# nju-ee/MODE-2022

Measured on AMD Instinct MI355X. Metric: ERP stereo pairs/sec (512x1024, 192 disp) fwd+bwd, higher is better.
Workload: dtype fp32 storage/accumulate; products: 2xfp16 split (22-bit, per-tensor 2^k scale, 3 MFMAs) in the stride-1 3x3x3 / spherical / 3x3 layers incl. gradients (DESIGN 3u/3v); 3xbf16 split (24-bit, 6 MFMAs) in the stride-2 / transposed 3x3x3 layers and the polar spherical tiles (3j-3l); fp32 MFMA in the 32->; 1 GPU; ModeDisparity(192,Sphere,1024x512 Cassini) fwd+bwd+Adam step, batch 2/GPU (BASELINE configs[2]); global_batch=2, conv_arith=bf16x6, init=recipe state, seed 1 (tests/golden/recipe.py), parallelism=dp1

## Files before the change

mode-2022_amd/csrc/conv2d_split_wgrad.hip:

```cpp
#include "common.h"

#include "bn_internal.h"
#include "conv3d_internal.h"
#include "split_arith.h"

namespace {

using namespace mode::split;

constexpr int NT = 256;
constexpr int RING = 12;
constexpr int XROWP = 40;
constexpr int XPIECE = RING * XROWP;
constexpr int XCS = 3 * XPIECE + 8;
constexpr int XALL = 32 * XCS;
constexpr int GPIECE = 4 * 32;
constexpr int GCS = 3 * GPIECE + 8;
constexpr int GBUF = 32 * GCS;
constexpr size_t TILE_BYTES = (size_t)(XALL + 2 * GBUF) * 2;
constexpr size_t SUM_BYTES = (size_t)3 * 9 * 1024 * sizeof(float);
constexpr size_t LDS_BYTES = TILE_BYTES > SUM_BYTES ? TILE_BYTES : SUM_BYTES;
constexpr int GIT = 32 * 4 * 16 / NT;

template <int DIL, bool F16>
__global__ __launch_bounds__(NT) void conv2d_bww_split_kernel(const float* __restrict__ gy, const float* __restrict__ x,
                                                              float* __restrict__ part, mode::Wgrad2SplitDims d,
                                                              const float* __restrict__ amax_g, const float* __restrict__ amax_x) {
  constexpr int NPC = Arith<F16>::NP;
  float sg = 1.f, sx = 1.f, unscale = 1.f;
  if (F16) {
    sg = f16_scale_of(mode::absmax_load(amax_g));
    sx = f16_scale_of(mode::absmax_load(amax_x));
    unscale = (1.f / sg) * (1.f / sx);
  }
  constexpr int NP = (32 + 2 * DIL) / 2;
  constexpr int XIT = (32 * 4 * NP + NT - 1) / NT;
  extern __shared__ __attribute__((aligned(16))) uint16_t lds[];
  uint16_t* xl = lds;
  uint16_t* gl = lds + XALL;
  const int s = blockIdx.x, ob = blockIdx.y, cb = blockIdx.z;
  const int tid = threadIdx.x, wave = tid >> 6, lane = tid & 63, half = lane >> 5;
  const int HWi = d.H * d.W;

  f32x16 acc[9];
#pragma unroll
  for (int t = 0; t < 9; ++t) acc[t] = (f32x16){0};

  int x_c[XIT], x_row[XIT], x_wp[XIT], g_o[GIT], g_row[GIT], g_wp[GIT];
#pragma unroll
  for (int k = 0; k < XIT; ++k) {
    const int item = min(tid + k * NT, 32 * 4 * NP - 1);
    x_wp[k] = item % NP;
    x_row[k] = (item / NP) % 4;
    x_c[k] = item / (NP * 4);
  }
#pragma unroll
  for (int k = 0; k < GIT; ++k) {
    const int item = tid + k * NT;
    g_wp[k] = item % 16;
    g_row[k] = (item / 16) % 4;
    g_o[k] = item / 64;
  }
  const float* xb = x;
  const float* gb = gy;
  float xr[XIT][2], gr[GIT][2];
  constexpr unsigned kHalfOOB = 0x40000000u;
  unsigned xo0[XIT], xo1[XIT], go0[GIT], go1[GIT];
  int xdst[XIT], gdst[GIT];
#pragma unroll
  for (int k = 0; k < XIT; ++k) xdst[k] = x_c[k] * XCS + 2 * x_wp[k];
#pragma unroll
  for (int k = 0; k < GIT; ++k) gdst[k] = g_o[k] * GCS + g_row[k] * 32 + 2 * g_wp[k];
  auto unit_begin = [&](int w0) {
#pragma unroll
    for (int k = 0; k < XIT; ++k) {
      const int gw = w0 - DIL + 2 * x_wp[k];
      const unsigned cok = (unsigned)(cb * 32 + x_c[k] < d.Ci);
      const unsigned base = 4u * (unsigned)(x_c[k] * HWi + x_row[k] * d.W + gw);
      xo0[k] = (cok & (unsigned)((unsigned)gw < (unsigned)d.W)) ? base : kHalfOOB;
      xo1[k] = (cok & (unsigned)((unsigned)(gw + 1) < (unsigned)d.W)) ? base + 4u : kHalfOOB;
    }
#pragma unroll
    for (int k = 0; k < GIT; ++k) {
      const int gw = w0 + 2 * g_wp[k];
      const unsigned ook = (unsigned)(ob * 32 + g_o[k] < d.Co);
      const unsigned base = 4u * (unsigned)(g_o[k] * HWi + g_row[k] * d.W + gw);
      go0[k] = (ook & (unsigned)(gw < d.W)) ? base : kHalfOOB;
      go1[k] = (ook & (unsigned)(gw + 1 < d.W)) ? base + 4u : kHalfOOB;
    }
  };
  const unsigned block_bytes = 128u * (unsigned)HWi;
  auto load_x = [&](int k, int r0) {
    const __amdgpu_buffer_rsrc_t rs = buf_rsrc(xb, block_bytes);
    const unsigned ro = (unsigned)(r0 + x_row[k]) < (unsigned)d.H ? (unsigned)(4 * r0 * d.W) : kHalfOOB;
    xr[k][0] = buf_load_f32(rs, xo0[k] + ro, 0);
    xr[k][1] = buf_load_f32(rs, xo1[k] + ro, 0);
  };
  auto commit_x = [&](int k, int r0, int slot0) {
    uint32_t p1, p2, p3;
    const float v0 = xr[k][0], v1 = xr[k][1];
    int sl = slot0 + x_row[k];
    sl = sl >= RING ? sl - RING : sl;
    uint32_t* dst = reinterpret_cast<uint32_t*>(xl + xdst[k] + sl * XROWP);
    if constexpr (F16) {
      split2_f16_pinned(v0 * sx, v1 * sx, p1, p2);
    } else {
      split3_bf16_pinned(v0, v1, p1, p2, p3);
      dst[XPIECE] = p3;
    }
    dst[0] = p1;
    dst[XPIECE / 2] = p2;
  };
  auto load_g = [&](int k, int r0) {
    const __amdgpu_buffer_rsrc_t rs = buf_rsrc(gb, block_bytes);
    const unsigned ro = r0 + g_row[k] < d.H ? (unsigned)(4 * r0 * d.W) : kHalfOOB;
    gr[k][0] = buf_load_f32(rs, go0[k] + ro, 0);
    gr[k][1] = buf_load_f32(rs, go1[k] + ro, 0);
  };
  auto commit_g = [&](int k, int r0, int buf) {
    uint32_t p1, p2, p3;
    const float v0 = gr[k][0], v1 = gr[k][1];
    uint32_t* dst = reinterpret_cast<uint32_t*>(gl + buf * GBUF + gdst[k]);
    if constexpr (F16) {
      split2_f16_pinned(v0 * sg, v1 * sg, p1, p2);
    } else {
      split3_bf16_pinned(v0, v1, p1, p2, p3);
      dst[GPIECE] = p3;
    }
    dst[0] = p1;
    dst[GPIECE / 2] = p2;
  };

  for (int u = xcd_remap(s, d.S); u < d.units; u += d.S) {
    int t = u;
    const int run = t % d.nRun;
    t /= d.nRun;
    const int wt = t % d.nWt;
    const int b = t / d.nWt;
    const int g_lo = run * d.run_groups, g_hi = min(d.nGroups, g_lo + d.run_groups);
    xb = x + ((long long)b * d.Ci + cb * 32) * HWi;
    gb = gy + ((long long)b * d.Co + ob * 32) * HWi;
    unit_begin(wt * 32);

    const int h_first = g_lo * 4;
#pragma unroll 1
    for (int pass = 0; pass < 2; ++pass) {
#pragma unroll
      for (int k = 0; k < XIT; ++k) load_x(k, h_first - DIL + 4 * pass);
#pragma unroll
      for (int k = 0; k < XIT; ++k) commit_x(k, h_first - DIL + 4 * pass, 4 * pass);
    }
#pragma unroll
    for (int k = 0; k < GIT; ++k) load_g(k, h_first);
#pragma unroll
    for (int k = 0; k < GIT; ++k) commit_g(k, h_first, 0);
    lds_barrier();

    int sbase = 0;
#pragma unroll 1
    for (int g = g_lo; g < g_hi; ++g) {
      const int h0 = g * 4, gbuf = (g - g_lo) & 1;
      const int sfront = sbase + 8 >= RING ? sbase + 8 - RING : sbase + 8;
      int xrow[3];
#pragma unroll
      for (int kh = 0; kh < 3; ++kh) {
        int sl = sbase + wave + kh * DIL;
        sl = sl >= RING ? sl - RING : sl;
        xrow[kh] = (lane & 31) * XCS + sl * XROWP + 8 * half;
      }
      const uint16_t* ga = gl + gbuf * GBUF + (lane & 31) * GCS + wave * 32 + 8 * half;
      uint4 ra[2][3], rlo[2][3];
      uint2 rhi[2][3];
      auto read_stage = [&](int i) {
        const int ks = i / 3, kh = i % 3;
#pragma unroll
        for (int p = 0; p < NPC; ++p) {
          if (kh == 0) ra[ks][p] = *reinterpret_cast<const uint4*>(__builtin_assume_aligned(ga + p * GPIECE + 16 * ks, 16));
          const uint32_t* src = reinterpret_cast<const uint32_t*>(__builtin_assume_aligned(xl + xrow[kh] + p * XPIECE + 16 * ks, 16));
          rlo[i & 1][p] = *reinterpret_cast<const uint4*>(src);
          rhi[i & 1][p] = *reinterpret_cast<const uint2*>(src + 4);
        }
      };
      read_stage(0);
#pragma unroll
      for (int i = 0; i < 6; ++i) {
        const int ks = i / 3, kh = i % 3;
        if (i + 1 < 6) read_stage(i + 1);
        if (i < 3) {
#pragma unroll
          for (int k = 3 * i; k < 3 * i + 3; ++k) load_x(k, h0 - DIL + 8);
#pragma unroll
          for (int k = (GIT * i) / 3; k < (GIT * (i + 1)) / 3; ++k) load_g(k, h0 + 4);
          if (!F16) __builtin_amdgcn_sched_barrier(0);
        } else {
#pragma unroll
          for (int k = 3 * (i - 3); k < 3 * (i - 3) + 3; ++k) commit_x(k, h0 - DIL + 8, sfront);
#pragma unroll
          for (int k = (GIT * (i - 3)) / 3; k < (GIT * (i - 2)) / 3; ++k) commit_g(k, h0 + 4, gbuf ^ 1);
        }
        uint4 bq[3][3];
#pragma unroll
        for (int p = 0; p < NPC; ++p) {
          const uint4 lo = rlo[i & 1][p];
          const uint2 hi = rhi[i & 1][p];
          const uint32_t dw[6] = {lo.x, lo.y, lo.z, lo.w, hi.x, hi.y};
          constexpr uint32_t SEL_MID = 0x05040302u, SEL_HI = 0x07060504u;
#pragma unroll
          for (int kw = 0; kw < 3; ++kw) {
            const int sh = kw * DIL;
            if (sh == 0) {
              bq[kw][p] = lo;
            } else {
              const int sd = sh == 4 ? 1 : 0;
              const uint32_t sel = (sh & 1) ? SEL_MID : SEL_HI;
              bq[kw][p] = make_uint4(__builtin_amdgcn_perm(dw[sd + 1], dw[sd], sel), __builtin_amdgcn_perm(dw[sd + 2], dw[sd + 1], sel),
                                     __builtin_amdgcn_perm(dw[sd + 3], dw[sd + 2], sel), __builtin_amdgcn_perm(dw[sd + 4], dw[sd + 3], sel));
            }
          }
        }
        if constexpr (F16) {
#define MODE_SPLIT_TERM(PA, PB) \
  _Pragma("unroll") for (int kw = 0; kw < 3; ++kw) acc[3 * kh + kw] = mfma_f16(ra[ks][PA], bq[kw][PB], acc[3 * kh + kw]);
          MODE_SPLIT_TERM(1, 0)
          MODE_SPLIT_TERM(0, 1)
          MODE_SPLIT_TERM(0, 0)
#undef MODE_SPLIT_TERM
        } else {
#define MODE_SPLIT_TERM(PA, PB) \
  _Pragma("unroll") for (int kw = 0; kw < 3; ++kw) acc[3 * kh + kw] = mfma_bf16(ra[ks][PA], bq[kw][PB], acc[3 * kh + kw]);
          MODE_SPLIT_TERM(2, 0)
          MODE_SPLIT_TERM(0, 2)
          MODE_SPLIT_TERM(1, 1)
          MODE_SPLIT_TERM(1, 0)
          MODE_SPLIT_TERM(0, 1)
          MODE_SPLIT_TERM(0, 0)
#undef MODE_SPLIT_TERM
        }
#pragma unroll
        for (int j = 0; j < (F16 ? 9 : 18); ++j) {
          __builtin_amdgcn_sched_group_barrier(0x008, 1, 0);
          if (F16) {
            __builtin_amdgcn_sched_group_barrier(0x002, 6, 0);
            if (i < 3) {
              __builtin_amdgcn_sched_group_barrier(0x020, 2, 0);
              __builtin_amdgcn_sched_group_barrier(0x080, 1, 0);
            } else {
              __builtin_amdgcn_sched_group_barrier(0x080, 2, 0);
            }
          } else {
            __builtin_amdgcn_sched_group_barrier(0x002, 7, 0);
            __builtin_amdgcn_sched_group_barrier(0x100, 1, 0);
            __builtin_amdgcn_sched_group_barrier(0x200, 2, 0);
          }
        }
        __builtin_amdgcn_sched_barrier(0);
      }
      sbase = sbase + 4 >= RING ? sbase + 4 - RING : sbase + 4;
      lds_barrier();
    }
  }

  float* sums = reinterpret_cast<float*>(lds);
  if (wave > 0) {
#pragma unroll
    for (int tap = 0; tap < 9; ++tap)
#pragma unroll
      for (int q = 0; q < 16; ++q) sums[((wave - 1) * 9 + tap) * 1024 + q * 64 + lane] = acc[tap][q];
  }
  __syncthreads();
  if (wave == 0) {
    float* pb = part + (((long long)s * d.MTo + ob) * d.MTc + cb) * (9 * 1024);
#pragma unroll
    for (int tap = 0; tap < 9; ++tap)
#pragma unroll
      for (int q = 0; q < 16; ++q) {
        const int i = (q & 3) + 8 * (q >> 2) + 4 * half;
        const float v = ((acc[tap][q] + sums[tap * 1024 + q * 64 + lane]) + sums[(9 + tap) * 1024 + q * 64 + lane]) +
                        sums[(18 + tap) * 1024 + q * 64 + lane];
        pb[tap * 1024 + i * 32 + (lane & 31)] = F16 ? v * unscale : v;
      }
  }
}

}

namespace mode {

int conv2d_bww_split_launch(const float* gy, const float* x, float* part, const Wgrad2SplitDims& d, int dilation, hipStream_t st,
                            const char* who, const float* amax_g, const float* amax_x) {
#define MODE_C2W_LAUNCH(DILV, F16V)                                                                                              \
  {                                                                                                                              \
    int rc = allow_lds(conv2d_bww_split_kernel<DILV, F16V>, LDS_BYTES, who);                                                     \
    if (rc != MODE_OK) return rc;                                                                                                \
    hipLaunchKernelGGL((conv2d_bww_split_kernel<DILV, F16V>), dim3(d.S, d.MTo, d.MTc), dim3(NT), LDS_BYTES, st, gy, x, part, d, amax_g, \
                       amax_x);                                                                                                  \
  }
  if (dilation == 1) {
    if (amax_g) MODE_C2W_LAUNCH(1, true) else MODE_C2W_LAUNCH(1, false)
  } else {
    if (amax_g) MODE_C2W_LAUNCH(2, true) else MODE_C2W_LAUNCH(2, false)
  }
#undef MODE_C2W_LAUNCH
  return check_launch(who);
}

}
```

mode-2022_amd/csrc/conv2d_wgrad.hip:

```cpp
#include "common.h"
#include "conv3d_internal.h"

namespace {

typedef float f32x16 __attribute__((ext_vector_type(16)));
constexpr int NT = 256;
constexpr int TH = 4;

__device__ __forceinline__ f32x16 mfma32(float a, float b, f32x16 c) {
  return __builtin_amdgcn_mfma_f32_32x32x2f32(a, b, c, 0, 0, 0);
}

struct W2Dims {
  int B, Ci, Co, H, W;
  int nHt, nWt, T, S, MTo, MTc;
};

template <int DIL>
struct Geo {
  static constexpr int XR = TH + 2 * DIL, XW = 32 + 2 * DIL;
  static constexpr int XPLANE = (XR * XW) | 1;
  static constexpr int GPLANE = TH * 32 + 1;
  static constexpr size_t LDS = (size_t)(32 * XPLANE + 32 * GPLANE) * sizeof(float);
};

template <int DIL>
__global__ __launch_bounds__(NT, 2) void conv2d_bwd_weight_kernel(const float* __restrict__ gy, const float* __restrict__ x,
                                                                  float* __restrict__ part, W2Dims d) {
  using G = Geo<DIL>;
  constexpr int XR = G::XR, XW = G::XW, XPLANE = G::XPLANE, GPLANE = G::GPLANE;
  constexpr int NXM = 4 * XR;
  constexpr int NHALO = 32 * XR * 2 * DIL;
  constexpr int NXH = (NHALO + NT - 1) / NT;
  extern __shared__ __attribute__((aligned(16))) float lds[];
  float* xl = lds;
  float* gl = lds + 32 * XPLANE;
  const int s = blockIdx.x, ob = blockIdx.y, cb = blockIdx.z;
  const int tid = threadIdx.x, wave = tid >> 6, lane = tid & 63;
  const int hwv = tid >> 5, l32 = tid & 31;
  const int HW = d.H * d.W;

  f32x16 acc[9];
#pragma unroll
  for (int t = 0; t < 9; ++t) acc[t] = (f32x16){0};

  float px[NXM], ph[NXH], pg[16];
  unsigned chan_ok = 0, gchan_ok = 0;
#pragma unroll
  for (int q = 0; q < 4; ++q) {
    chan_ok |= (cb * 32 + hwv + 8 * q < d.Ci ? 1u : 0u) << q;
    gchan_ok |= (ob * 32 + hwv + 8 * q < d.Co ? 1u : 0u) << q;
  }

  auto halo_geom = [&](int k, int& c, int& r, int& col) {
    const int e = k * NT + tid;
    const int cr = e / (2 * DIL), j = e - cr * (2 * DIL);
    c = cr / XR;
    r = cr - c * XR;
    col = j < DIL ? j : 32 + j;
    return e < NHALO;
  };

  auto prefetch = [&](int tt, int& h0, int& w0) {
    int t = tt;
    const int wt = t % d.nWt;
    t /= d.nWt;
    const int ht = t % d.nHt;
    const int b = t / d.nHt;
    w0 = wt * 32;
    h0 = ht * TH;
    const float* xb = x + ((long long)b * d.Ci + cb * 32) * (long long)HW;
    const float* gb = gy + ((long long)b * d.Co + ob * 32) * (long long)HW;
    const int gw = w0 + l32;
    const bool wok = gw < d.W;
#pragma unroll
    for (int jj = 0; jj < NXM; ++jj) {
      const int q = jj / XR, r = jj % XR;
      const int gh = h0 + r - DIL;
      const bool ok = ((chan_ok >> q) & 1) && wok && gh >= 0 && gh < d.H;
      px[jj] = xb[(unsigned)(ok ? (hwv + 8 * q) * HW + gh * d.W + gw : 0)];
    }
#pragma unroll
    for (int k = 0; k < NXH; ++k) {
      int c, r, col;
      const bool in = halo_geom(k, c, r, col);
      const int gh = h0 + r - DIL, gwh = w0 + col - DIL;
      const bool ok = in && cb * 32 + c < d.Ci && gh >= 0 && gh < d.H && gwh >= 0 && gwh < d.W;
      ph[k] = xb[(unsigned)(ok ? c * HW + gh * d.W + gwh : 0)];
    }
#pragma unroll
    for (int j = 0; j < 16; ++j) {
      const int q = j >> 2, r = j & 3;
      const int gh = h0 + r;
      const bool ok = ((gchan_ok >> q) & 1) && wok && gh < d.H;
      pg[j] = gb[(unsigned)(ok ? (hwv + 8 * q) * HW + gh * d.W + gw : 0)];
    }
  };
  auto store = [&](int h0, int w0) {
    const bool wok = w0 + l32 < d.W;
    float* xrow = xl + hwv * XPLANE + DIL + l32;
#pragma unroll
    for (int jj = 0; jj < NXM; ++jj) {
      const int q = jj / XR, r = jj % XR;
      const int gh = h0 + r - DIL;
      const bool ok = ((chan_ok >> q) & 1) && wok && gh >= 0 && gh < d.H;
      xrow[q * 8 * XPLANE + r * XW] = ok ? px[jj] : 0.f;
    }
#pragma unroll
    for (int k = 0; k < NXH; ++k) {
      int c, r, col;
      const bool in = halo_geom(k, c, r, col);
      const int gh = h0 + r - DIL, gwh = w0 + col - DIL;
      const bool ok = cb * 32 + c < d.Ci && gh >= 0 && gh < d.H && gwh >= 0 && gwh < d.W;
      if (in) xl[c * XPLANE + r * XW + col] = ok ? ph[k] : 0.f;
    }
    float* grow = gl + hwv * GPLANE + l32;
#pragma unroll
    for (int j = 0; j < 16; ++j) {
      const int q = j >> 2, r = j & 3;
      const bool ok = ((gchan_ok >> q) & 1) && wok && h0 + r < d.H;
      grow[q * 8 * GPLANE + r * 32] = ok ? pg[j] : 0.f;
    }
  };

  const int s_x = xcd_remap(s, d.S);
  int h0 = 0, w0 = 0, nh0 = 0, nw0 = 0;
  if (s_x < d.T) prefetch(s_x, nh0, nw0);
  const float* ap = gl + (lane & 31) * GPLANE + wave * 32 + (lane >> 5);
  const float* bp = xl + (lane & 31) * XPLANE + wave * XW + (lane >> 5);
  for (int tt = s_x; tt < d.T; tt += d.S) {
    h0 = nh0;
    w0 = nw0;
    store(h0, w0);
    __syncthreads();
    if (tt + d.S < d.T) prefetch(tt + d.S, nh0, nw0);
    __builtin_amdgcn_sched_barrier(0);
    float a_n = ap[0], b_n[9];
#pragma unroll
    for (int t = 0; t < 9; ++t) b_n[t] = bp[(t / 3) * DIL * XW + (t % 3) * DIL];
#pragma unroll
    for (int ks = 0; ks < 16; ++ks) {
      const float a = a_n;
      float bb[9];
#pragma unroll
      for (int t = 0; t < 9; ++t) bb[t] = b_n[t];
      if (ks + 1 < 16) {
        a_n = ap[2 * (ks + 1)];
#pragma unroll
        for (int t = 0; t < 9; ++t) b_n[t] = bp[2 * (ks + 1) + (t / 3) * DIL * XW + (t % 3) * DIL];
      }
      __builtin_amdgcn_sched_barrier(0);
#pragma unroll
      for (int t = 0; t < 9; ++t) acc[t] = mfma32(a, bb[t], acc[t]);
    }
    __syncthreads();
  }

  float* red = lds;
  float* pb = part + (((long long)s * d.MTo + ob) * d.MTc + cb) * (9 * 1024);
#pragma unroll
  for (int t3 = 0; t3 < 3; ++t3) {
#pragma unroll
    for (int u = 0; u < 3; ++u)
#pragma unroll
      for (int q = 0; q < 16; ++q) {
        const int i = (q & 3) + 8 * (q >> 2) + 4 * (lane >> 5);
        red[(u * 4 + wave) * 1024 + i * 32 + (lane & 31)] = acc[t3 * 3 + u][q];
      }
    __syncthreads();
    for (int idx = tid; idx < 3 * 1024; idx += NT) {
      const int u = idx >> 10, e = idx & 1023;
      const float* r4 = red + u * 4096 + e;
      pb[(t3 * 3 + u) * 1024 + e] = (r4[0] + r4[1024]) + (r4[2048] + r4[3072]);
    }
    __syncthreads();
  }
}

__global__ __launch_bounds__(256) void reduce_gw2d(const float* __restrict__ part, float* __restrict__ gw, W2Dims d, int accumulate) {
  __shared__ float sh[8][33];
  const long long stride = (long long)d.MTo * d.MTc * 9 * 1024;
  const int el = threadIdx.x & 31, g = threadIdx.x >> 5;
  const long long e = (long long)blockIdx.x * 32 + el;
  float a0 = 0.f, a1 = 0.f;
  if (e < stride) {
    const float* p = part + e;
    int s = g;
    for (; s + 8 < d.S; s += 16) {
      a0 += p[(long long)s * stride];
      a1 += p[(long long)(s + 8) * stride];
    }
    if (s < d.S) a0 += p[(long long)s * stride];
  }
  sh[g][el] = a0 + a1;
  __syncthreads();
  if (g == 0 && e < stride) {
    const float sum = ((sh[0][el] + sh[1][el]) + (sh[2][el] + sh[3][el])) + ((sh[4][el] + sh[5][el]) + (sh[6][el] + sh[7][el]));
    const int j = (int)(e & 31), i = (int)((e >> 5) & 31);
    long long r = e >> 10;
    const int tap = (int)(r % 9);
    r /= 9;
    const int cb = (int)(r % d.MTc), ob = (int)(r / d.MTc);
    const int o = ob * 32 + i, c = cb * 32 + j;
    if (o < d.Co && c < d.Ci) {
      float* q = gw + ((long long)o * d.Ci + c) * 9 + tap;
      *q = accumulate ? *q + sum : sum;
    }
  }
}

void make_dims(W2Dims& d, int B, int Ci, int H, int W, int Co) {
  d.B = B; d.Ci = Ci; d.Co = Co; d.H = H; d.W = W;
  d.nHt = mode::cdiv(H, TH);
  d.nWt = mode::cdiv(W, 32);
  d.T = B * d.nHt * d.nWt;
  d.MTo = mode::cdiv(Co, 32);
  d.MTc = mode::cdiv(Ci, 32);
  int S = mode::cdiv(2 * kNumCU, d.MTo * d.MTc);
  if (S > d.T) S = d.T;
  d.S = S < 1 ? 1 : S;
}

template <int DIL>
int launch(const float* gy, const float* x, float* workspace, const W2Dims& d, hipStream_t st, const char* who) {
  const size_t lds = std::max(Geo<DIL>::LDS, (size_t)3 * 4 * 1024 * sizeof(float));
  int rc = mode::allow_lds(conv2d_bwd_weight_kernel<DIL>, lds, who);
  if (rc != MODE_OK) return rc;
  hipLaunchKernelGGL(conv2d_bwd_weight_kernel<DIL>, dim3(d.S, d.MTo, d.MTc), dim3(NT), lds, st, gy, x, workspace, d);
  return mode::check_launch(who);
}

}

extern "C" size_t mode_conv2d_bwd_weight_workspace_bytes(int B, int Ci, int H, int W, int Co) {
  if (B <= 0 || Ci <= 0 || Co <= 0 || H <= 0 || W <= 0) return 0;
  W2Dims d;
  make_dims(d, B, Ci, H, W, Co);
  return (size_t)d.S * d.MTo * d.MTc * 9 * 1024 * sizeof(float);
}

extern "C" int mode_conv2d_bwd_weight(const float* gy, const float* x, float* gw, float* workspace, int B, int Ci, int H, int W, int Co,
                                      int dilation, int accumulate, mode_stream_t stream) {
  const char* who = "mode_conv2d_bwd_weight";
  MODE_REQUIRE(B >= 0 && Ci > 0 && Co > 0 && H > 0 && W > 0, MODE_ERR_BAD_ARG, "%s: non-positive size", who);
  MODE_REQUIRE(dilation == 1 || dilation == 2, MODE_ERR_UNSUPPORTED, "%s: dilation %d not implemented (1 or 2)", who, dilation);
  MODE_REQUIRE((long long)std::max(Ci, Co) * H * W < (1ll << 29), MODE_ERR_UNSUPPORTED, "%s: a sample larger than 2^29 elements", who);
  hipStream_t st = mode::as_stream(stream);
  if (B == 0) {
    if (!accumulate) return mode::zero_floats(gw, (size_t)Co * Ci * 9, st, "mode_conv2d_bwd_weight");
    return MODE_OK;
  }
  MODE_REQUIRE(gy && x && gw && workspace, MODE_ERR_BAD_ARG, "%s: null pointer", who);
  W2Dims d;
  make_dims(d, B, Ci, H, W, Co);
  int rc = dilation == 1 ? launch<1>(gy, x, workspace, d, st, who) : launch<2>(gy, x, workspace, d, st, who);
  if (rc != MODE_OK) return rc;
  hipLaunchKernelGGL(reduce_gw2d, dim3(mode::cdiv((long long)d.MTo * d.MTc * 9 * 1024, 32)), dim3(256), 0, st, workspace, gw, d, accumulate);
  return mode::check_launch("mode_conv2d_bwd_weight(reduce)");
}

static int conv2d_bwd_weight_split(const char* who, const float* gy, const float* x, const float* amax_g, const float* amax_x, float* gw,
                                   float* workspace, int B, int Ci, int H, int W, int Co, int dilation, int accumulate, mode_stream_t stream);

extern "C" int mode_conv2d_bwd_weight_split(const float* gy, const float* x, float* gw, float* workspace, int B, int Ci, int H, int W, int Co,
                                            int dilation, int accumulate, mode_stream_t stream) {
  return conv2d_bwd_weight_split("mode_conv2d_bwd_weight_split", gy, x, nullptr, nullptr, gw, workspace, B, Ci, H, W, Co, dilation, accumulate,
                                 stream);
}

extern "C" int mode_conv2d_bwd_weight_split_f16(const float* gy, const float* x, const float* amax_g, const float* amax_x, float* gw,
                                                float* workspace, int B, int Ci, int H, int W, int Co, int dilation, int accumulate,
                                                mode_stream_t stream) {
  MODE_REQUIRE(amax_g && amax_x, MODE_ERR_BAD_ARG, "mode_conv2d_bwd_weight_split_f16: null maximum");
  return conv2d_bwd_weight_split("mode_conv2d_bwd_weight_split_f16", gy, x, amax_g, amax_x, gw, workspace, B, Ci, H, W, Co, dilation, accumulate,
                                 stream);
}

static int conv2d_bwd_weight_split(const char* who, const float* gy, const float* x, const float* amax_g, const float* amax_x, float* gw,
                                   float* workspace, int B, int Ci, int H, int W, int Co, int dilation, int accumulate, mode_stream_t stream) {
  MODE_REQUIRE(B >= 0 && Ci > 0 && Co > 0 && H > 0 && W > 0, MODE_ERR_BAD_ARG, "%s: non-positive size", who);
  MODE_REQUIRE(dilation == 1 || dilation == 2, MODE_ERR_UNSUPPORTED, "%s: dilation %d not implemented (1 or 2)", who, dilation);
  MODE_REQUIRE(mode_conv2d_split_shape_supported(Ci, Co, H, W, dilation, 2) == 1, MODE_ERR_UNSUPPORTED,
               "%s: %dx%d at %d -> %d channels is beyond the 32-bit offsets of the split kernel (mode_conv2d_split_shape_supported)", who, H, W, Ci,
               Co);
  hipStream_t st = mode::as_stream(stream);
  if (B == 0) {
    if (!accumulate) return mode::zero_floats(gw, (size_t)Co * Ci * 9, st, "mode_conv2d_bwd_weight");
    return MODE_OK;
  }
  MODE_REQUIRE(gy && x && gw && workspace, MODE_ERR_BAD_ARG, "%s: null pointer", who);
  W2Dims d;
  make_dims(d, B, Ci, H, W, Co);
  mode::Wgrad2SplitDims q;
  q.Ci = Ci; q.Co = Co; q.H = H; q.W = W;
  q.nWt = d.nWt; q.MTo = d.MTo; q.MTc = d.MTc;
  q.nGroups = mode::cdiv(H, 4);
  int S = mode::cdiv(kNumCU, d.MTo * d.MTc);
  int run = q.nGroups;
  while (run > 4 && (long long)B * d.nWt * mode::cdiv(q.nGroups, run) < S) run = mode::cdiv(run, 2);
  q.run_groups = run;
  q.nRun = mode::cdiv(q.nGroups, run);
  q.units = B * d.nWt * q.nRun;
  if (S > q.units) S = q.units;
  if (S > d.S) S = d.S;
  q.S = d.S = S;
  int rc = mode::conv2d_bww_split_launch(gy, x, workspace, q, dilation, st, who, amax_g, amax_x);
  if (rc != MODE_OK) return rc;
  hipLaunchKernelGGL(reduce_gw2d, dim3(mode::cdiv((long long)d.MTo * d.MTc * 9 * 1024, 32)), dim3(256), 0, st, workspace, gw, d, accumulate);
  return mode::check_launch("mode_conv2d_bwd_weight_split(reduce)");
}
```

mode-2022_amd/csrc/conv3d_internal.h:

```cpp
#pragma once
#include "common.h"
#include "size_contracts.h"

namespace mode {

int conv3d_co1_fwd(const float* x, const float* w, float* y, int B, int Ci, int D, int H, int W, hipStream_t st, const char* who);

int conv3d_co1_fwd_small(const float* x, const float* w, float* y, int B, int Ci, int D, int H, int W, hipStream_t st, const char* who);

int conv3d_co1_bwd_data(const float* gy, const float* w, float* gx, int B, int Ci, int D, int H, int W, hipStream_t st, const char* who);

size_t conv3d_co1_bwd_weight_workspace_floats(int B, int Ci, int D, int H, int W);
int conv3d_co1_bwd_weight(const float* gy, const float* x, float* gw, float* workspace, int B, int Ci, int D, int H, int W,
                          int accumulate, hipStream_t st, const char* who);

bool conv3d_split_supported(int K, int rows);
size_t conv3d_split_wpack_floats(int K, int rows);
int conv3d_split_stat_partials();
int conv3d_s1_split(const float* x, const float* w, float* y, float* wpack, int B, int K, int rows, int D, int H, int W, int flip,
                    hipStream_t st, const char* who, const mode_bn_epilogue* bn, float* stats = nullptr, const float* acc_in = nullptr,
                    const float* amax_x = nullptr, const float* amax_w = nullptr, float* amax_y = nullptr);

int abs_max(const float* x, long long n, float* out, hipStream_t st, const char* who);
int abs_max_batch(const float* const* ptrs, const long long* sizes, int n, float* out, hipStream_t st, const char* who);

bool conv3d_s2_split_supported(int K, int rows);
size_t conv3d_s2_split_wpack_floats(int K, int rows);
int conv3d_s2_split(const float* x, const float* w, float* y, float* wpack, int B, int K, int rows, int D, int H, int W, hipStream_t st,
                    const char* who, const mode_bn_epilogue* bn = nullptr, float* amax_y = nullptr);

bool deconv3d_split_supported(int K, int Co);
bool deconv3d_split_bn_supported(int K, int Co);
size_t deconv3d_split_wpack_floats(int K, int Co);
int deconv3d_split(const float* x, const float* w, float* y, float* wpack, int B, int K, int Co, int D, int H, int W, hipStream_t st,
                   const char* who, const mode_bn_epilogue* bn = nullptr, const float* acc_in = nullptr, float* amax_y = nullptr);

struct WgradSplitDims {
  int Ci, Co, D, H, W;
  int nWt, nHt, nDc, ring_dc, units;
  int S, MTo, MTc;
};
int conv3d_bww_split_launch(const float* gy, const float* x, float* part, const WgradSplitDims& d, hipStream_t st, const char* who,
                            const float* amax_g = nullptr, const float* amax_x = nullptr);

struct WgradS2SplitDims {
  int Ci, Co, D, H, W, Do, Ho, Wo;
  int nWt, nDc, ring_dc, units;
  int S, MTo, MTc;
};
int conv3d_bww_s2_split_launch(const float* gy, const float* x, float* part, const WgradS2SplitDims& d, hipStream_t st, const char* who);

bool conv2d_split_supported(int K, int rows, int dilation);
size_t conv2d_split_wpack_floats(int K, int rows);
int conv2d_split_run(const float* x, const float* w, float* y, float* wpack, int B, int K, int rows, int H, int W, int dilation, int flip,
                     hipStream_t st, const char* who, const mode_bn_epilogue* bn, const float* acc_in = nullptr,
                     const float* amax_x = nullptr, const float* amax_w = nullptr, float* amax_y = nullptr);

struct Wgrad2SplitDims {
  int Ci, Co, H, W;
  int nWt, nGroups, run_groups, nRun, units;
  int S, MTo, MTc;
};
int conv2d_bww_split_launch(const float* gy, const float* x, float* part, const Wgrad2SplitDims& d, int dilation, hipStream_t st,
                            const char* who, const float* amax_g = nullptr, const float* amax_x = nullptr);

}
```

Before: 37.60 pairs/s.

## Add 64-output-channel block to 2D split weight-gradient kernel for fp16 path

Adds a ROWS=64 variant of the 2D conv weight-gradient kernel. Each block computes two 32-row output-channel tiles, reusing the staged x tile across both and halving x loads per output. Part of the 18 accumulators are placed in ordinary VGPRs through inline-asm MFMA, and the schedule-group barriers are retuned. The host picks 64 rows by default when fp16 is used and Co is a multiple of 64, falling back to 32 when the run split would be too short. The trade-offs are higher register pressure and fewer blocks in flight.

```diff
diff --git a/mode-2022_amd/csrc/conv2d_split_wgrad.hip b/mode-2022_amd/csrc/conv2d_split_wgrad.hip
--- a/mode-2022_amd/csrc/conv2d_split_wgrad.hip
+++ b/mode-2022_amd/csrc/conv2d_split_wgrad.hip
@@ -12,21 +12,45 @@
 constexpr int RING = 12;
 constexpr int XROWP = 40;
 constexpr int XPIECE = RING * XROWP;
-constexpr int XCS = 3 * XPIECE + 8;
-constexpr int XALL = 32 * XCS;
 constexpr int GPIECE = 4 * 32;
-constexpr int GCS = 3 * GPIECE + 8;
-constexpr int GBUF = 32 * GCS;
-constexpr size_t TILE_BYTES = (size_t)(XALL + 2 * GBUF) * 2;
 constexpr size_t SUM_BYTES = (size_t)3 * 9 * 1024 * sizeof(float);
-constexpr size_t LDS_BYTES = TILE_BYTES > SUM_BYTES ? TILE_BYTES : SUM_BYTES;
-constexpr int GIT = 32 * 4 * 16 / NT;
-
-template <int DIL, bool F16>
+constexpr int GIT32 = 32 * 4 * 16 / NT;
+
+template <int ROWS>
+struct Lay {
+  static constexpr int NPL = ROWS == 64 ? 2 : 3;
+  static constexpr int XCS = NPL * XPIECE + 8;
+  static constexpr int XALL = 32 * XCS;
+  static constexpr int GCS = NPL * GPIECE + 8;
+  static constexpr int GBUF = ROWS * GCS;
+  static constexpr size_t TILE_BYTES = (size_t)(XALL + 2 * GBUF) * 2;
+  static constexpr size_t LDS_BYTES = TILE_BYTES > SUM_BYTES ? TILE_BYTES : SUM_BYTES;
+};
+
+constexpr int kVgprAccFirst = 16;
+__device__ __forceinline__ f32x16 mfma_f16_vgpr(uint4 a, uint4 b, f32x16 c) {
+  asm("s_nop 1\n\tv_mfma_f32_32x32x16_f16 %0, %1, %2, %0" : "+v"(c) : "v"(__builtin_bit_cast(f16x8, a)), "v"(__builtin_bit_cast(f16x8, b)));
+  return c;
+}
+template <bool SPLIT_HOMES>
+__device__ __forceinline__ f32x16 mfma_f16_at(int t, uint4 a, uint4 b, f32x16 c) {
+  return SPLIT_HOMES && t >= kVgprAccFirst ? mfma_f16_vgpr(a, b, c) : mfma_f16(a, b, c);
+}
+__device__ __forceinline__ void settle_vgpr_acc(f32x16& c0, f32x16& c1) { asm volatile("s_nop 15" : "+v"(c0), "+v"(c1)); }
+
+template <int DIL, bool F16, int ROWS>
 __global__ __launch_bounds__(NT) void conv2d_bww_split_kernel(const float* __restrict__ gy, const float* __restrict__ x,
                                                               float* __restrict__ part, mode::Wgrad2SplitDims d,
                                                               const float* __restrict__ amax_g, const float* __restrict__ amax_x) {
+  static_assert(ROWS == 32 || (ROWS == 64 && F16), "the 64-row block is built for the two-piece arithmetic");
+  using L = Lay<ROWS>;
+  constexpr int XCS = L::XCS, XALL = L::XALL, GCS = L::GCS, GBUF = L::GBUF;
+  constexpr int NB = ROWS / 32;
+  constexpr int GIT = NB * GIT32;
+  constexpr bool QUAD = ROWS == 64;
+  constexpr int GN = QUAD ? 1 : GIT32;
   constexpr int NPC = Arith<F16>::NP;
+  static_assert(NPC <= L::NPL, "pieces beyond the layout");
   float sg = 1.f, sx = 1.f, unscale = 1.f;
   if (F16) {
     sg = f16_scale_of(mode::absmax_load(amax_g));
@@ -38,70 +62,93 @@
   extern __shared__ __attribute__((aligned(16))) uint16_t lds[];
   uint16_t* xl = lds;
   uint16_t* gl = lds + XALL;
-  const int s = blockIdx.x, ob = blockIdx.y, cb = blockIdx.z;
+  const int s = blockIdx.x, ob = blockIdx.y * NB, cb = blockIdx.z;
   const int tid = threadIdx.x, wave = tid >> 6, lane = tid & 63, half = lane >> 5;
   const int HWi = d.H * d.W;
 
-  f32x16 acc[9];
-#pragma unroll
-  for (int t = 0; t < 9; ++t) acc[t] = (f32x16){0};
-
-  int x_c[XIT], x_row[XIT], x_wp[XIT], g_o[GIT], g_row[GIT], g_wp[GIT];
-#pragma unroll
-  for (int k = 0; k < XIT; ++k) {
-    const int item = min(tid + k * NT, 32 * 4 * NP - 1);
-    x_wp[k] = item % NP;
-    x_row[k] = (item / NP) % 4;
-    x_c[k] = item / (NP * 4);
-  }
-#pragma unroll
-  for (int k = 0; k < GIT; ++k) {
-    const int item = tid + k * NT;
-    g_wp[k] = item % 16;
-    g_row[k] = (item / 16) % 4;
-    g_o[k] = item / 64;
-  }
+  f32x16 acc[NB * 9];
+#pragma unroll
+  for (int t = 0; t < NB * 9; ++t) acc[t] = (f32x16){0};
+
+  constexpr int XN = QUAD ? 2 : XIT;
+  constexpr int NTAIL = NP - 16;
+  static_assert(!QUAD || (XIT == 9 && 32 * 4 * NTAIL <= NT), "eight quads and one tail item per thread");
+  auto xi = [](int k) { return QUAD ? (k < 8 ? 0 : 1) : k; };
+  int x_c[XN], x_row[XN], x_wp[XN], g_o[GN], g_row[GN], g_wp[GN];
+  int xdst[XN], gdst[GN];
+  auto items_of = [&](int tid) {
+    if constexpr (QUAD) {
+      x_wp[0] = tid % 16;
+      x_c[0] = (tid / 16) % 4;
+      x_row[0] = tid / 64;
+      const int item = min(tid, 32 * 4 * NTAIL - 1);
+      x_wp[1] = 16 + item % NTAIL;
+      x_row[1] = (item / NTAIL) % 4;
+      x_c[1] = item / (NTAIL * 4);
+    } else {
+#pragma unroll
+      for (int k = 0; k < XIT; ++k) {
+        const int item = min(tid + k * NT, 32 * 4 * NP - 1);
+        x_wp[k] = item % NP;
+        x_row[k] = (item / NP) % 4;
+        x_c[k] = item / (NP * 4);
+      }
+    }
+#pragma unroll
+    for (int k = 0; k < GN; ++k) {
+      const int item = tid + k * NT;
+      g_wp[k] = item % 16;
+      g_row[k] = (item / 16) % 4;
+      g_o[k] = item / 64;
+    }
+#pragma unroll
+    for (int k = 0; k < XN; ++k) xdst[k] = x_c[k] * XCS + 2 * x_wp[k];
+#pragma unroll
+    for (int k = 0; k < GN; ++k) gdst[k] = g_o[k] * GCS + g_row[k] * 32 + 2 * g_wp[k];
+  };
+  items_of(tid);
   const float* xb = x;
   const float* gb = gy;
   float xr[XIT][2], gr[GIT][2];
   constexpr unsigned kHalfOOB = 0x40000000u;
-  unsigned xo0[XIT], xo1[XIT], go0[GIT], go1[GIT];
-  int xdst[XIT], gdst[GIT];
-#pragma unroll
-  for (int k = 0; k < XIT; ++k) xdst[k] = x_c[k] * XCS + 2 * x_wp[k];
-#pragma unroll
-  for (int k = 0; k < GIT; ++k) gdst[k] = g_o[k] * GCS + g_row[k] * 32 + 2 * g_wp[k];
+  unsigned xo0[XN], xo1[XN], go0[GN], go1[GN];
   auto unit_begin = [&](int w0) {
 #pragma unroll
-    for (int k = 0; k < XIT; ++k) {
+    for (int k = 0; k < XN; ++k) {
       const int gw = w0 - DIL + 2 * x_wp[k];
-      const unsigned cok = (unsigned)(cb * 32 + x_c[k] < d.Ci);
+      const unsigned cok = QUAD && k == 0 ? 1u : (unsigned)(cb * 32 + x_c[k] < d.Ci);
       const unsigned base = 4u * (unsigned)(x_c[k] * HWi + x_row[k] * d.W + gw);
       xo0[k] = (cok & (unsigned)((unsigned)gw < (unsigned)d.W)) ? base : kHalfOOB;
       xo1[k] = (cok & (unsigned)((unsigned)(gw + 1) < (unsigned)d.W)) ? base + 4u : kHalfOOB;
     }
 #pragma unroll
-    for (int k = 0; k < GIT; ++k) {
+    for (int k = 0; k < GN; ++k) {
       const int gw = w0 + 2 * g_wp[k];
-      const unsigned ook = (unsigned)(ob * 32 + g_o[k] < d.Co);
+      const unsigned ook = ROWS == 64 ? 1u : (unsigned)(ob * 32 + g_o[k] < d.Co);
       const unsigned base = 4u * (unsigned)(g_o[k] * HWi + g_row[k] * d.W + gw);
       go0[k] = (ook & (unsigned)(gw < d.W)) ? base : kHalfOOB;
       go1[k] = (ook & (unsigned)(gw + 1 < d.W)) ? base + 4u : kHalfOOB;
     }
   };
   const unsigned block_bytes = 128u * (unsigned)HWi;
+  unsigned quad_bytes[8];
+#pragma unroll
+  for (int k = 0; k < 8; ++k)
+    quad_bytes[k] = QUAD ? __builtin_amdgcn_readfirstlane(4u * (unsigned)HWi * (unsigned)min(max(d.Ci - cb * 32 - 4 * k, 0), 4)) : 0u;
   auto load_x = [&](int k, int r0) {
-    const __amdgpu_buffer_rsrc_t rs = buf_rsrc(xb, block_bytes);
-    const unsigned ro = (unsigned)(r0 + x_row[k]) < (unsigned)d.H ? (unsigned)(4 * r0 * d.W) : kHalfOOB;
-    xr[k][0] = buf_load_f32(rs, xo0[k] + ro, 0);
-    xr[k][1] = buf_load_f32(rs, xo1[k] + ro, 0);
+    const int kk = xi(k);
+    const __amdgpu_buffer_rsrc_t rs = QUAD && k < 8 ? buf_rsrc(xb + (long long)(4 * k) * HWi, quad_bytes[k % 8]) : buf_rsrc(xb, block_bytes);
+    const unsigned ro = (unsigned)(r0 + x_row[kk]) < (unsigned)d.H ? (unsigned)(4 * r0 * d.W) : kHalfOOB;
+    xr[k][0] = buf_load_f32(rs, xo0[kk] + ro, 0);
+    xr[k][1] = buf_load_f32(rs, xo1[kk] + ro, 0);
   };
   auto commit_x = [&](int k, int r0, int slot0) {
     uint32_t p1, p2, p3;
+    const int kk = xi(k);
     const float v0 = xr[k][0], v1 = xr[k][1];
-    int sl = slot0 + x_row[k];
+    int sl = slot0 + x_row[kk];
     sl = sl >= RING ? sl - RING : sl;
-    uint32_t* dst = reinterpret_cast<uint32_t*>(xl + xdst[k] + sl * XROWP);
+    uint32_t* dst = reinterpret_cast<uint32_t*>(xl + xdst[kk] + (QUAD && k < 8 ? 4 * k * XCS : 0) + sl * XROWP);
     if constexpr (F16) {
       split2_f16_pinned(v0 * sx, v1 * sx, p1, p2);
     } else {
@@ -112,15 +159,17 @@
     dst[XPIECE / 2] = p2;
   };
   auto load_g = [&](int k, int r0) {
-    const __amdgpu_buffer_rsrc_t rs = buf_rsrc(gb, block_bytes);
-    const unsigned ro = r0 + g_row[k] < d.H ? (unsigned)(4 * r0 * d.W) : kHalfOOB;
-    gr[k][0] = buf_load_f32(rs, go0[k] + ro, 0);
-    gr[k][1] = buf_load_f32(rs, go1[k] + ro, 0);
+    const __amdgpu_buffer_rsrc_t rs = buf_rsrc(gb + (long long)(k / GIT32) * 32 * HWi, block_bytes);
+    const int kk = ROWS == 64 ? 0 : k;
+    const unsigned so = ROWS == 64 ? 16u * (unsigned)(k % GIT32) * (unsigned)HWi : 0u;
+    const unsigned ro = r0 + g_row[kk] < d.H ? (unsigned)(4 * r0 * d.W) : kHalfOOB;
+    gr[k][0] = buf_load_f32(rs, go0[kk] + ro, so);
+    gr[k][1] = buf_load_f32(rs, go1[kk] + ro, so);
   };
   auto commit_g = [&](int k, int r0, int buf) {
     uint32_t p1, p2, p3;
     const float v0 = gr[k][0], v1 = gr[k][1];
-    uint32_t* dst = reinterpret_cast<uint32_t*>(gl + buf * GBUF + gdst[k]);
+    uint32_t* dst = reinterpret_cast<uint32_t*>(gl + buf * GBUF + (ROWS == 64 ? 4 * k * GCS + gdst[0] : gdst[k]));
     if constexpr (F16) {
       split2_f16_pinned(v0 * sg, v1 * sg, p1, p2);
     } else {
@@ -169,13 +218,17 @@
         xrow[kh] = (lane & 31) * XCS + sl * XROWP + 8 * half;
       }
       const uint16_t* ga = gl + gbuf * GBUF + (lane & 31) * GCS + wave * 32 + 8 * half;
-      uint4 ra[2][3], rlo[2][3];
+      uint4 ra[2][NB][3], rlo[2][3];
       uint2 rhi[2][3];
       auto read_stage = [&](int i) {
         const int ks = i / 3, kh = i % 3;
 #pragma unroll
         for (int p = 0; p < NPC; ++p) {
-          if (kh == 0) ra[ks][p] = *reinterpret_cast<const uint4*>(__builtin_assume_aligned(ga + p * GPIECE + 16 * ks, 16));
+          if (kh == 0) {
+#pragma unroll
+            for (int nb = 0; nb < NB; ++nb)
+              ra[ks][nb][p] = *reinterpret_cast<const uint4*>(__builtin_assume_aligned(ga + nb * 32 * GCS + p * GPIECE + 16 * ks, 16));
+          }
           const uint32_t* src = reinterpret_cast<const uint32_t*>(__builtin_assume_aligned(xl + xrow[kh] + p * XPIECE + 16 * ks, 16));
           rlo[i & 1][p] = *reinterpret_cast<const uint4*>(src);
           rhi[i & 1][p] = *reinterpret_cast<const uint2*>(src + 4);
@@ -219,15 +272,17 @@
           }
         }
         if constexpr (F16) {
-#define MODE_SPLIT_TERM(PA, PB) \
-  _Pragma("unroll") for (int kw = 0; kw < 3; ++kw) acc[3 * kh + kw] = mfma_f16(ra[ks][PA], bq[kw][PB], acc[3 * kh + kw]);
+#define MODE_SPLIT_TERM(PA, PB)                                  \
+  _Pragma("unroll") for (int kw = 0; kw < 3; ++kw)               \
+  _Pragma("unroll") for (int nb = 0; nb < NB; ++nb)              \
+    acc[9 * nb + 3 * kh + kw] = mfma_f16_at<(ROWS == 64)>(9 * nb + 3 * kh + kw, ra[ks][nb][PA], bq[kw][PB], acc[9 * nb + 3 * kh + kw]);
           MODE_SPLIT_TERM(1, 0)
           MODE_SPLIT_TERM(0, 1)
           MODE_SPLIT_TERM(0, 0)
 #undef MODE_SPLIT_TERM
         } else {
 #define MODE_SPLIT_TERM(PA, PB) \
-  _Pragma("unroll") for (int kw = 0; kw < 3; ++kw) acc[3 * kh + kw] = mfma_bf16(ra[ks][PA], bq[kw][PB], acc[3 * kh + kw]);
+  _Pragma("unroll") for (int kw = 0; kw < 3; ++kw) acc[3 * kh + kw] = mfma_bf16(ra[ks][0][PA], bq[kw][PB], acc[3 * kh + kw]);
           MODE_SPLIT_TERM(2, 0)
           MODE_SPLIT_TERM(0, 2)
           MODE_SPLIT_TERM(1, 1)
@@ -237,9 +292,17 @@
 #undef MODE_SPLIT_TERM
         }
 #pragma unroll
-        for (int j = 0; j < (F16 ? 9 : 18); ++j) {
+        for (int j = 0; j < (F16 ? NB * 9 : 18); ++j) {
           __builtin_amdgcn_sched_group_barrier(0x008, 1, 0);
-          if (F16) {
+          if (ROWS == 64) {
+            __builtin_amdgcn_sched_group_barrier(0x002, 5, 0);
+            if (i < 3) {
+              __builtin_amdgcn_sched_group_barrier(0x020, 1, 0);
+              if (j % 2 == 0) __builtin_amdgcn_sched_group_barrier(0x080, 1, 0);
+            } else {
+              __builtin_amdgcn_sched_group_barrier(0x080, 1, 0);
+            }
+          } else if (F16) {
             __builtin_amdgcn_sched_group_barrier(0x002, 6, 0);
             if (i < 3) {
               __builtin_amdgcn_sched_group_barrier(0x020, 2, 0);
@@ -260,25 +323,30 @@
     }
   }
 
+  if constexpr (ROWS == 64) settle_vgpr_acc(acc[kVgprAccFirst], acc[kVgprAccFirst + 1]);
   float* sums = reinterpret_cast<float*>(lds);
-  if (wave > 0) {
-#pragma unroll
-    for (int tap = 0; tap < 9; ++tap)
-#pragma unroll
-      for (int q = 0; q < 16; ++q) sums[((wave - 1) * 9 + tap) * 1024 + q * 64 + lane] = acc[tap][q];
-  }
-  __syncthreads();
-  if (wave == 0) {
-    float* pb = part + (((long long)s * d.MTo + ob) * d.MTc + cb) * (9 * 1024);
-#pragma unroll
-    for (int tap = 0; tap < 9; ++tap)
-#pragma unroll
-      for (int q = 0; q < 16; ++q) {
-        const int i = (q & 3) + 8 * (q >> 2) + 4 * half;
-        const float v = ((acc[tap][q] + sums[tap * 1024 + q * 64 + lane]) + sums[(9 + tap) * 1024 + q * 64 + lane]) +
-                        sums[(18 + tap) * 1024 + q * 64 + lane];
-        pb[tap * 1024 + i * 32 + (lane & 31)] = F16 ? v * unscale : v;
-      }
+#pragma unroll
+  for (int nb = 0; nb < NB; ++nb) {
+    if (nb > 0) __syncthreads();
+    if (wave > 0) {
+#pragma unroll
+      for (int tap = 0; tap < 9; ++tap)
+#pragma unroll
+        for (int q = 0; q < 16; ++q) sums[((wave - 1) * 9 + tap) * 1024 + q * 64 + lane] = acc[9 * nb + tap][q];
+    }
+    __syncthreads();
+    if (wave == 0) {
+      float* pb = part + (((long long)s * d.MTo + ob + nb) * d.MTc + cb) * (9 * 1024);
+#pragma unroll
+      for (int tap = 0; tap < 9; ++tap)
+#pragma unroll
+        for (int q = 0; q < 16; ++q) {
+          const int i = (q & 3) + 8 * (q >> 2) + 4 * half;
+          const float v = ((acc[9 * nb + tap][q] + sums[tap * 1024 + q * 64 + lane]) + sums[(9 + tap) * 1024 + q * 64 + lane]) +
+                          sums[(18 + tap) * 1024 + q * 64 + lane];
+          pb[tap * 1024 + i * 32 + (lane & 31)] = F16 ? v * unscale : v;
+        }
+    }
   }
 }
 
@@ -287,18 +355,22 @@
 namespace mode {
 
 int conv2d_bww_split_launch(const float* gy, const float* x, float* part, const Wgrad2SplitDims& d, int dilation, hipStream_t st,
-                            const char* who, const float* amax_g, const float* amax_x) {
-#define MODE_C2W_LAUNCH(DILV, F16V)                                                                                              \
+                            const char* who, const float* amax_g, const float* amax_x, int rows) {
+  if (rows != 32 && !(rows == 64 && amax_g && d.Co % 64 == 0)) {
+    set_error("%s: a %d-row block at %d output channels%s", who, rows, d.Co, amax_g ? "" : " without maxima");
+    return MODE_ERR_BAD_ARG;
+  }
+#define MODE_C2W_LAUNCH(DILV, F16V, ROWSV)                                                                                       \
   {                                                                                                                              \
-    int rc = allow_lds(conv2d_bww_split_kernel<DILV, F16V>, LDS_BYTES, who);                                                     \
+    int rc = allow_lds(conv2d_bww_split_kernel<DILV, F16V, ROWSV>, Lay<ROWSV>::LDS_BYTES, who);                                  \
     if (rc != MODE_OK) return rc;                                                                                                \
-    hipLaunchKernelGGL((conv2d_bww_split_kernel<DILV, F16V>), dim3(d.S, d.MTo, d.MTc), dim3(NT), LDS_BYTES, st, gy, x, part, d, amax_g, \
-                       amax_x);                                                                                                  \
+    hipLaunchKernelGGL((conv2d_bww_split_kernel<DILV, F16V, ROWSV>), dim3(d.S, d.MTo / (ROWSV / 32), d.MTc), dim3(NT),           \
+                       Lay<ROWSV>::LDS_BYTES, st, gy, x, part, d, amax_g, amax_x);                                               \
   }
   if (dilation == 1) {
-    if (amax_g) MODE_C2W_LAUNCH(1, true) else MODE_C2W_LAUNCH(1, false)
+    if (rows == 64) MODE_C2W_LAUNCH(1, true, 64) else if (amax_g) MODE_C2W_LAUNCH(1, true, 32) else MODE_C2W_LAUNCH(1, false, 32)
   } else {
-    if (amax_g) MODE_C2W_LAUNCH(2, true) else MODE_C2W_LAUNCH(2, false)
+    if (rows == 64) MODE_C2W_LAUNCH(2, true, 64) else if (amax_g) MODE_C2W_LAUNCH(2, true, 32) else MODE_C2W_LAUNCH(2, false, 32)
   }
 #undef MODE_C2W_LAUNCH
   return check_launch(who);
diff --git a/mode-2022_amd/csrc/conv2d_wgrad.hip b/mode-2022_amd/csrc/conv2d_wgrad.hip
--- a/mode-2022_amd/csrc/conv2d_wgrad.hip
+++ b/mode-2022_amd/csrc/conv2d_wgrad.hip
@@ -1,5 +1,7 @@
 #include "common.h"
 #include "conv3d_internal.h"
+
+#include <cstdlib>
 
 namespace {
 
@@ -276,6 +278,16 @@
                                  stream);
 }
 
+constexpr int kRows64MinRun = 16;
+static int bww2d_rows(bool f16, int Co, bool* forced) {
+  *forced = false;
+  if (!f16 || Co % 64 != 0) return 32;
+  const char* e = std::getenv("MODE_BWW2D_ROWS");
+  const int v = e ? std::atoi(e) : 0;
+  *forced = v == 64;
+  return v == 32 ? 32 : 64;
+}
+
 static int conv2d_bwd_weight_split(const char* who, const float* gy, const float* x, const float* amax_g, const float* amax_x, float* gw,
                                    float* workspace, int B, int Ci, int H, int W, int Co, int dilation, int accumulate, mode_stream_t stream) {
   MODE_REQUIRE(B >= 0 && Ci > 0 && Co > 0 && H > 0 && W > 0, MODE_ERR_BAD_ARG, "%s: non-positive size", who);
@@ -295,16 +307,22 @@
   q.Ci = Ci; q.Co = Co; q.H = H; q.W = W;
   q.nWt = d.nWt; q.MTo = d.MTo; q.MTc = d.MTc;
   q.nGroups = mode::cdiv(H, 4);
-  int S = mode::cdiv(kNumCU, d.MTo * d.MTc);
-  int run = q.nGroups;
-  while (run > 4 && (long long)B * d.nWt * mode::cdiv(q.nGroups, run) < S) run = mode::cdiv(run, 2);
+  bool forced;
+  int rows = bww2d_rows(amax_g != nullptr, Co, &forced);
+  int S, run;
+  for (;; rows = 32) {
+    S = mode::cdiv(kNumCU, d.MTo / (rows / 32) * d.MTc);
+    run = q.nGroups;
+    while (run > 4 && (long long)B * d.nWt * mode::cdiv(q.nGroups, run) < S) run = mode::cdiv(run, 2);
+    if (rows == 32 || forced || run >= kRows64MinRun || q.nGroups < kRows64MinRun) break;
+  }
   q.run_groups = run;
   q.nRun = mode::cdiv(q.nGroups, run);
   q.units = B * d.nWt * q.nRun;
   if (S > q.units) S = q.units;
   if (S > d.S) S = d.S;
   q.S = d.S = S;
-  int rc = mode::conv2d_bww_split_launch(gy, x, workspace, q, dilation, st, who, amax_g, amax_x);
+  int rc = mode::conv2d_bww_split_launch(gy, x, workspace, q, dilation, st, who, amax_g, amax_x, rows);
   if (rc != MODE_OK) return rc;
   hipLaunchKernelGGL(reduce_gw2d, dim3(mode::cdiv((long long)d.MTo * d.MTc * 9 * 1024, 32)), dim3(256), 0, st, workspace, gw, d, accumulate);
   return mode::check_launch("mode_conv2d_bwd_weight_split(reduce)");
diff --git a/mode-2022_amd/csrc/conv3d_internal.h b/mode-2022_amd/csrc/conv3d_internal.h
--- a/mode-2022_amd/csrc/conv3d_internal.h
+++ b/mode-2022_amd/csrc/conv3d_internal.h
@@ -62,6 +62,6 @@
   int S, MTo, MTc;
 };
 int conv2d_bww_split_launch(const float* gy, const float* x, float* part, const Wgrad2SplitDims& d, int dilation, hipStream_t st,
-                            const char* who, const float* amax_g = nullptr, const float* amax_x = nullptr);
+                            const char* who, const float* amax_g = nullptr, const float* amax_x = nullptr, int rows = 32);
 
 }
```

Result: no change. 37.78 pairs/s, median of 6 (+0.5%).
